# allenai/gpv-1

Measured on AMD Instinct MI355X. Metric: images/sec/node (train step, 480x640, bs32/GPU), higher is better.
Workload: dtype bf16; 1 GPU; GPV-1 (ResNet-50 + 6+6 DETR layers, 100 queries, RoI head, BERT-base, 3 co-attention, 3 text-decoder layers, V=10000) CocoCaptioning-only train step, dropout 0.1, AdamW; global_batch=32, image=480x640, parallelism=dp1

## Files before the change

gpv-1_amd/csrc/gemm_glds_tt.hip:

```cpp
#include "gemm_common.h"

namespace gpvk {
namespace {


typedef __attribute__((address_space(3))) void lds_void_t;
typedef const __attribute__((address_space(1))) void glb_void_t;

__device__ __forceinline__ bf16x8 tr_frag(const unsigned char* p) {
  typedef short __attribute__((ext_vector_type(4))) s16x4;
  typedef __attribute__((address_space(3))) s16x4 lds_s16x4;
  s16x4 a = __builtin_amdgcn_ds_read_tr16_b64_v4i16((lds_s16x4*)(p));
  s16x4 b = __builtin_amdgcn_ds_read_tr16_b64_v4i16((lds_s16x4*)(p + 4 * ROWBYTES));
  typedef short __attribute__((ext_vector_type(8))) s16x8;
  s16x8 r = {a[0], a[1], a[2], a[3], b[0], b[1], b[2], b[3]};
  return __builtin_bit_cast(bf16x8, r);
}

template <bool CONV, int ABL = 0>
__device__ __forceinline__ void glds_tt_core(const GemmK& p, int tile, int ksplit) {
  extern __shared__ __attribute__((aligned(256))) unsigned char smem[];
  const int tid = threadIdx.x, lane = tid & 63, wave = tid >> 6;
  const int wm = wave >> 1, wn = wave & 1;
  const ConvGeom& g = p.cg;
  const int tm = tile / p.tilesN, tn = tile - tm * p.tilesN;
  const int row0 = tm * TBM, col0 = tn * TBN;
  const int kt_total = (p.K + TBK - 1) / TBK;
  const int kt0 = ksplit * p.kt_per_split;
  const int kt1 = min(kt_total, kt0 + p.kt_per_split);
  if (kt0 >= kt1) return;

  int c0 = 0, dh = 0, dw = 0;
  if constexpr (CONV) {
    const int tap = col0 / g.Cin;
    c0 = col0 - tap * g.Cin;
    const int tap_r = tap / g.KW, tap_s = tap - tap_r * g.KW;
    dh = tap_r - g.PH; dw = tap_s - g.PW;
  }

  int px_b = 0, px_oh = 0, px_ow = 0, adv_q = 0, adv_r = 0;
  if constexpr (CONV) {
    const int k = kt0 * TBK + lane;
    px_b = k / (g.OH * g.OW);
    const int rem = k - px_b * (g.OH * g.OW);
    px_oh = rem / g.OW;
    px_ow = rem - px_oh * g.OW;
    adv_q = TBK / g.OW; adv_r = TBK - adv_q * g.OW;
  }

  constexpr int OOB = 0x7ffffff0;
  const int lrow = lane >> 4;
  const int chunk01 = (lane & 15) ^ (2 * lrow);
  const auto rsA = __builtin_amdgcn_make_buffer_rsrc(const_cast<void*>(p.A), (short)0, OOB, 0x00020000);
  const auto rsB = __builtin_amdgcn_make_buffer_rsrc(const_cast<void*>(p.B), (short)0, OOB, 0x00020000);
  int a_vo[4], b_vo[4];
#pragma unroll
  for (int j = 0; j < 4; ++j) {
    const int r = wave * 16 + j * 4 + lrow;
    const int ch = chunk01 ^ ((j >> 1) * 8);
    a_vo[j] = (r * (int)p.lda + row0 + ch * 8) * 2;
    b_vo[j] = CONV ? (c0 + ch * 8) * 2 : (r * (int)p.ldb + col0 + ch * 8) * 2;
  }
  auto bload = [&](const decltype(rsA)& rs, int voff, int soff, unsigned char* l) {
    __builtin_amdgcn_raw_ptr_buffer_load_lds(rs, (lds_void_t*)l, 16, voff, soff, 0, 0);
  };

  auto issue = [&](int kt, int stage) {
    unsigned char* sa = smem + stage * TSTAGE + wave * (4 * 1024);
    unsigned char* sb = sa + OP_BYTES;
    const bool full = (kt + 1) * TBK <= p.K;
    if constexpr (CONV) {
      int off;
      {
        const int ih = px_oh * g.SH + dh, iw = px_ow * g.SW + dw;
        const bool ok = (unsigned)ih < (unsigned)g.IH && (unsigned)iw < (unsigned)g.IW && kt * TBK + lane < p.K;
        off = ok ? ((px_b * g.IH + ih) * g.IW + iw) * g.Cs * 2 : OOB;
        px_ow += adv_r;
        const int c = px_ow >= g.OW ? 1 : 0;
        px_ow -= c ? g.OW : 0;
        px_oh += adv_q + c;
        const int c2 = px_oh >= g.OH ? 1 : 0;
        px_oh -= c2 ? g.OH : 0;
        px_b += c2;
      }
#pragma unroll
      for (int j = 0; j < 4; ++j)
        bload(rsB, __shfl(off, wave * 16 + j * 4 + lrow) + b_vo[j], 0, sb + j * 1024);
    } else {
#pragma unroll
      for (int j = 0; j < 4; ++j) {
        const bool ok = full || kt * TBK + wave * 16 + j * 4 + lrow < p.K;
        bload(rsB, ok ? b_vo[j] : OOB, kt * TBK * (int)p.ldb * 2, sb + j * 1024);
      }
    }
#pragma unroll
    for (int j = 0; j < 4; ++j) {
      const bool ok = full || kt * TBK + wave * 16 + j * 4 + lrow < p.K;
      bload(rsA, ok ? a_vo[j] : OOB, kt * TBK * (int)p.lda * 2, sa + j * 1024);
    }
  };

  f32x4 acc[4][4];
#pragma unroll
  for (int i = 0; i < 4; ++i)
#pragma unroll
    for (int j = 0; j < 4; ++j) acc[i][j] = f32x4{0.f, 0.f, 0.f, 0.f};

  const int li = lane & 15, fg = lane >> 4;
  const int fq = (li >> 2) | ((fg & 1) << 2);
  const int f_row = (8 * fg + (li >> 2)) * ROWBYTES + ((li & 3) >> 1) * 16 + (li & 1) * 8;
  int a_sl[4], b_sl[4];
#pragma unroll
  for (int i = 0; i < 4; ++i) {
    a_sl[i] = f_row + (((wm * 4 + i) ^ fq) << 5);
// ... 4 lines not shown
  f32x4 sacc[4];
#pragma unroll
  for (int i = 0; i < 4; ++i) sacc[i] = f32x4{0.f, 0.f, 0.f, 0.f};
  bf16x8 ones;
#pragma unroll
  for (int e = 0; e < 8; ++e) ones[e] = (bf16)1.0f;

  if (ABL == 5 || ABL == 6) {
    constexpr int AHEAD = ABL == 5 ? 2 : 3;
    for (int a = 0; a < AHEAD && kt0 + a < kt1; ++a) issue(kt0 + a, a & 1);
    for (int kt = kt0; kt < kt1; ++kt) {
      if (ABL == 5) asm volatile("s_waitcnt vmcnt(8)" ::: "memory"); else asm volatile("s_waitcnt vmcnt(16)" ::: "memory");
      __syncthreads();
      if (kt + AHEAD < kt1) issue(kt + AHEAD, kt & 1);
    }
    asm volatile("s_waitcnt vmcnt(0)" ::: "memory");
    return;
  }
  if (ABL != 3) issue(kt0, 0);
  for (int kt = kt0; kt < kt1; ++kt) {
    const int t = kt - kt0;
    asm volatile("s_waitcnt vmcnt(0)" ::: "memory");
    __syncthreads();
    if (ABL != 3 && kt + 1 < kt1) issue(ABL == 4 ? kt0 : kt + 1, (t + 1) & 1);
    const unsigned char* st = smem + (t & 1) * TSTAGE;
    if (ABL == 2 || ABL == 4) continue;
#pragma unroll
    for (int kk = 0; kk < 2; ++kk) {
      bf16x8 af[4], bfr[4];
#pragma unroll
      for (int j = 0; j < 4; ++j) bfr[j] = tr_frag(st + b_sl[j] + kk * 32 * ROWBYTES);
#pragma unroll
      for (int i = 0; i < 4; ++i) af[i] = tr_frag(st + a_sl[i] + kk * 32 * ROWBYTES);
      if (ABL == 1) {
#pragma unroll
        for (int i = 0; i < 4; ++i) asm volatile("" ::"v"(af[i]), "v"(bfr[i]));
        continue;
      }
#pragma unroll
      for (int i = 0; i < 4; ++i)
#pragma unroll
        for (int j = 0; j < 4; ++j) acc[i][j] = mfma16(bfr[j], af[i], acc[i][j]);
      if constexpr (!CONV) {
        if (do_sum) {
#pragma unroll
          for (int i = 0; i < 4; ++i) sacc[i] = mfma16(ones, af[i], sacc[i]);
        }
      }
    }
  }
  if constexpr (!CONV) {
    if (do_sum && fg == 0) {
#pragma unroll
      for (int i = 0; i < 4; ++i) atomicAdd(p.a_rowsum + row0 + wm * 64 + i * 16 + li, sacc[i][0]);
    }
  }

  const bool direct = p.ws == nullptr;
  float* Cp = direct ? reinterpret_cast<float*>(p.C) : p.ws + (int64_t)ksplit * p.M * p.N;
  const int64_t cpitch = direct ? p.ldc : p.N;
  float* ep = reinterpret_cast<float*>(smem);
  constexpr int EPITCH = TBN + 4;
#pragma unroll
  for (int half = 0; half < 2; ++half) {
    __syncthreads();
    if (wm == half) {
#pragma unroll
      for (int i = 0; i < 4; ++i)
#pragma unroll
        for (int j = 0; j < 4; ++j)
          *reinterpret_cast<f32x4*>(ep + (i * 16 + li) * EPITCH + wn * 64 + j * 16 + fg * 4) = acc[i][j];
    }
    __syncthreads();
#pragma unroll
    for (int q = 0; q < 8; ++q) {
      const int idx = tid + q * 256;
      const int r = idx >> 5, c4 = idx & 31;
      const int m = row0 + half * 64 + r;
      if (m >= p.M) continue;
      const float rs = p.rowscale ? p.rowscale[m] * p.alpha : p.alpha;
      float4 v = *reinterpret_cast<const float4*>(ep + r * EPITCH + c4 * 4);
      v.x *= rs; v.y *= rs; v.z *= rs; v.w *= rs;
      float4* dst = reinterpret_cast<float4*>(Cp + (int64_t)m * cpitch + col0 + c4 * 4);
      if (direct) { const float4 c = *dst; v.x += c.x; v.y += c.y; v.z += c.z; v.w += c.w; }
      *dst = v;
    }
  }
}

constexpr int W8_HALF = TBK * ROWBYTES;
constexpr int W8_BUF = 4 * W8_HALF;
constexpr int W8_LDS = 2 * W8_BUF;

typedef short __attribute__((ext_vector_type(4))) w8_s16x4;
typedef short __attribute__((ext_vector_type(8))) w8_s16x8;
template <int OFF>
__device__ __forceinline__ bf16x8 tr_frag_asm(uint32_t addr) {
  w8_s16x4 a, b;
  asm volatile("ds_read_b64_tr_b16 %0, %1 offset:%2" : "=v"(a) : "v"(addr), "n"(OFF) : "memory");
  asm volatile("ds_read_b64_tr_b16 %0, %1 offset:%2" : "=v"(b) : "v"(addr), "n"(OFF + 4 * ROWBYTES) : "memory");
  w8_s16x8 r = {a[0], a[1], a[2], a[3], b[0], b[1], b[2], b[3]};
  return __builtin_bit_cast(bf16x8, r);
}

template <bool CONV>
__device__ __forceinline__ void wg8_core(const GemmK& p, int tile, int ksplit) {
  extern __shared__ __attribute__((aligned(256))) unsigned char smem[];
  const int tid = threadIdx.x, lane = tid & 63;
  const int wave = __builtin_amdgcn_readfirstlane(tid >> 6);
  const int wm = wave >> 2, wn = wave & 3;
  const ConvGeom& g = p.cg;
  const int tm = tile / p.tilesN, tn = tile - tm * p.tilesN;
  const int row0 = tm * 256, col0 = tn * 256;
  const int kt_total = (p.K + TBK - 1) / TBK;
  const int kt0 = ksplit * p.kt_per_split;
  const int kt1 = min(kt_total, kt0 + p.kt_per_split);
  if (kt0 >= kt1) return;
  const int nkt = kt1 - kt0;

  constexpr int OOB = 0x7ffffff0;
  const int lrow = lane >> 4;
  const int myrow = wave * 8 + lrow;
  const int chunk = (lane & 15) ^ (2 * lrow) ^ (8 * (wave & 1));

  int c0 = 0, dh = 0, dw = 0, adv_q = 0, adv_r = 0;
  int px_b[2] = {0, 0}, px_oh[2] = {0, 0}, px_ow[2] = {0, 0}, px_k[2] = {0, 0};
  if constexpr (CONV) {
    const int tap = col0 / g.Cin;
    c0 = col0 - tap * g.Cin;
    const int tap_r = tap / g.KW, tap_s = tap - tap_r * g.KW;
    dh = tap_r - g.PH; dw = tap_s - g.PW;
    adv_q = TBK / g.OW; adv_r = TBK - adv_q * g.OW;
// ... 344 lines not shown
    __builtin_amdgcn_sched_barrier(0);
    issue01(t + 2, buf2);
    asm volatile("s_waitcnt vmcnt(10)" ::: "memory");
    mma(0, 0);
    if constexpr (BH == 2) { W8H_READ_B(2) } else { W8H_READ_A(2) }
    __builtin_amdgcn_sched_barrier(0);
    issue2(t + 2, buf2);
    asm volatile("s_waitcnt vmcnt(8)" ::: "memory");
    if constexpr (BH == 2) mma(0, 2); else mma(4, 0);
    buf = buf == 2 ? 0 : buf + 1;
    buf2 = buf2 == 2 ? 0 : buf2 + 1;
  }
#undef W8H_READ_A
#undef W8H_READ_B
  if (wm == 0) __builtin_amdgcn_s_barrier();
  asm volatile("s_waitcnt vmcnt(0)" ::: "memory");

  const bool direct = p.ws == nullptr;
  float* Cp = direct ? reinterpret_cast<float*>(p.C) : p.ws + (int64_t)ksplit * p.M * p.N;
  const int64_t cpitch = direct ? p.ldc : p.N;
#pragma unroll
  for (int i = 0; i < NI; ++i) {
    const int m = row0 + (i >> 2) * 128 + wm * 64 + (i & 3) * 16 + li;
    const float rs = p.rowscale ? p.rowscale[m] * p.alpha : p.alpha;
#pragma unroll
    for (int j = 0; j < NJ; ++j) {
      if (!hval[j >> 1]) continue;
      const int n = col0 + (j >> 1) * 128 + wn * 32 + (j & 1) * 16 + fg * 4;
      float4* dst = reinterpret_cast<float4*>(Cp + (int64_t)m * cpitch + n);
      float4 v = make_float4(acc[i][j][0] * rs, acc[i][j][1] * rs, acc[i][j][2] * rs, acc[i][j][3] * rs);
      if (direct) { const float4 c = *dst; v.x += c.x; v.y += c.y; v.z += c.z; v.w += c.w; }
      *dst = v;
    }
  }
}

template <bool CONV>
__device__ __forceinline__ void glds_tt_body(const GemmK& p) {
  const int gx = gridDim.x, nwg = gx * (int)gridDim.y, bid = (int)blockIdx.x + gx * (int)blockIdx.y;
  const int v = xcd_contiguous(bid, nwg);
  const int ksplit = v / gx;
  glds_tt_core<CONV>(p, v - ksplit * gx, ksplit);
}
__global__ __launch_bounds__(256) void glds_wgrad_kernel(GemmK p) { glds_tt_body<true>(p); }
__global__ __launch_bounds__(256) void glds_tt_kernel(GemmK p) { glds_tt_body<false>(p); }

struct GroupK {
  int n;
  int tile_start[GPV_TT_GROUP_MAX + 1];
  gpv_tt_problem prob[GPV_TT_GROUP_MAX];
};
static_assert(sizeof(GroupK) <= 4096, "kernel argument segment");

__global__ __launch_bounds__(256) void glds_tt_group_kernel(GroupK g) {
  const int bid = blockIdx.x;
  int pi = 0;
  while (pi + 1 < g.n && bid >= g.tile_start[pi + 1]) ++pi;
  const gpv_tt_problem& q = g.prob[pi];
  GemmK p{};
  p.A = q.A; p.B = q.B; p.C = q.C; p.a_rowsum = q.a_rowsum;
  p.M = q.M; p.N = q.N; p.K = q.K; p.lda = q.lda; p.ldb = q.ldb; p.ldc = q.ldc;
  p.alpha = 1.0f; p.ws = nullptr;
  p.tilesN = q.N / TBN;
  p.kt_per_split = (q.K + TBK - 1) / TBK;
  glds_tt_core<false>(p, bid - g.tile_start[pi], 0);
}

struct WgProb {
  const void* A; const void* B; float* C; const float* rowscale;
  int M, N, K, lda, ldc;
  int kt_per_split, tilesN, tiles;
  int unit_start;
  int direct;
  int64_t ws_off;
  int IH, IW, Cs, Cin, OH, OW, KH, KW, SH, SW, PH, PW;
};
static_assert(sizeof(WgProb) == 128, "descriptor size");
constexpr int WG_MAX = 28;
struct WgGroupK { int n; int pad; float* ws; WgProb prob[WG_MAX]; };
static_assert(sizeof(WgGroupK) <= 4096, "kernel argument segment");

template <int ABL>
__device__ __forceinline__ void wgrad_group_body(const WgGroupK& g) {
  const int nwg = gridDim.x, bid = blockIdx.x;
  const int v = xcd_contiguous(bid, nwg);
  int pi = 0;
  while (pi + 1 < g.n && v >= g.prob[pi + 1].unit_start) ++pi;
  const WgProb& q = g.prob[pi];
  GemmK p{};
  p.A = q.A; p.B = q.B; p.C = q.C; p.rowscale = q.rowscale;
  p.M = q.M; p.N = q.N; p.K = q.K; p.lda = q.lda; p.ldb = 0; p.ldc = q.ldc;
  p.alpha = 1.0f;
  p.ws = q.direct ? nullptr : g.ws + q.ws_off;
  p.tilesN = q.tilesN; p.kt_per_split = q.kt_per_split;
  p.cg.IH = q.IH; p.cg.IW = q.IW; p.cg.Cs = q.Cs; p.cg.Cin = q.Cin; p.cg.OH = q.OH; p.cg.OW = q.OW;
  p.cg.KH = q.KH; p.cg.KW = q.KW; p.cg.SH = q.SH; p.cg.SW = q.SW; p.cg.PH = q.PH; p.cg.PW = q.PW;
  const int u = v - q.unit_start;
  const int ksplit = u / q.tiles;
  glds_tt_core<true, ABL>(p, u - ksplit * q.tiles, ksplit);
}
__global__ __launch_bounds__(256) void glds_wgrad_group_kernel(WgGroupK g) { wgrad_group_body<0>(g); }
__global__ __launch_bounds__(512) void wg8_group_kernel(WgGroupK g) {
  const int nwg = gridDim.x, bid = blockIdx.x;
  const int v = xcd_contiguous(bid, nwg);
  int pi = 0;
  while (pi + 1 < g.n && v >= g.prob[pi + 1].unit_start) ++pi;
  const WgProb& q = g.prob[pi];
  GemmK p{};
  p.A = q.A; p.B = q.B; p.C = q.C; p.rowscale = q.rowscale;
  p.M = q.M; p.N = q.N; p.K = q.K; p.lda = q.lda; p.ldb = 0; p.ldc = q.ldc;
  p.alpha = 1.0f;
  p.ws = q.direct ? nullptr : g.ws + q.ws_off;
  p.tilesN = q.tilesN; p.kt_per_split = q.kt_per_split;
  p.cg.IH = q.IH; p.cg.IW = q.IW; p.cg.Cs = q.Cs; p.cg.Cin = q.Cin; p.cg.OH = q.OH; p.cg.OW = q.OW;
  p.cg.KH = q.KH; p.cg.KW = q.KW; p.cg.SH = q.SH; p.cg.SW = q.SW; p.cg.PH = q.PH; p.cg.PW = q.PW;
  const int u = v - q.unit_start;
  const int ksplit = u / q.tiles;
  wg8_core<true>(p, u - ksplit * q.tiles, ksplit);
}
__global__ __launch_bounds__(512) void wg8h_group_kernel(WgGroupK g) {
  const int nwg = gridDim.x, bid = blockIdx.x;
  const int v = xcd_contiguous(bid, nwg);
  int pi = 0;
  while (pi + 1 < g.n && v >= g.prob[pi + 1].unit_start) ++pi;
  const WgProb& q = g.prob[pi];
  GemmK p{};
  p.A = q.A; p.B = q.B; p.C = q.C; p.rowscale = q.rowscale;
  p.M = q.M; p.N = q.N; p.K = q.K; p.lda = q.lda; p.ldb = 0; p.ldc = q.ldc;
  p.alpha = 1.0f;
  p.ws = (q.direct & 1) ? nullptr : g.ws + q.ws_off;
  p.tilesN = q.tilesN; p.kt_per_split = q.kt_per_split;
  p.cg.IH = q.IH; p.cg.IW = q.IW; p.cg.Cs = q.Cs; p.cg.Cin = q.Cin; p.cg.OH = q.OH; p.cg.OW = q.OW;
  p.cg.KH = q.KH; p.cg.KW = q.KW; p.cg.SH = q.SH; p.cg.SW = q.SW; p.cg.PH = q.PH; p.cg.PW = q.PW;
  const int u = v - q.unit_start;
  const int ksplit = u / q.tiles;
  if (q.direct & 2) wg8h_core<2, 1>(p, u - ksplit * q.tiles, ksplit);
  else wg8h_core<1, 2>(p, u - ksplit * q.tiles, ksplit);
}
#ifdef GPV_TUNING
__global__ __launch_bounds__(256) void glds_wgrad_group_abl1_kernel(WgGroupK g) { wgrad_group_body<1>(g); }
__global__ __launch_bounds__(256) void glds_wgrad_group_abl2_kernel(WgGroupK g) { wgrad_group_body<2>(g); }
__global__ __launch_bounds__(256) void glds_wgrad_group_abl3_kernel(WgGroupK g) { wgrad_group_body<3>(g); }
__global__ __launch_bounds__(256) void glds_wgrad_group_abl4_kernel(WgGroupK g) { wgrad_group_body<4>(g); }
__global__ __launch_bounds__(256) void glds_wgrad_group_abl5_kernel(WgGroupK g) { wgrad_group_body<5>(g); }
__global__ __launch_bounds__(256) void glds_wgrad_group_abl6_kernel(WgGroupK g) { wgrad_group_body<6>(g); }
#endif

constexpr int W8L_PMAX = GPV_TT_GROUP_MAX, W8L_GMAX = 200;
struct W8LProb {
  const void* A; const void* B; float* C; float* a_rowsum;
  int MN, N, K, lda, ldb, ldc;
  int kt_per_split;
  int ws_off;
};
struct W8LGrp { unsigned short v_start; unsigned char prob, slice; };
struct W8LGroupK { int n_prob, n_grp, Q, pad; int cnt[8]; float* ws; W8LProb prob[W8L_PMAX]; W8LGrp grp[W8L_GMAX]; };
static_assert(sizeof(W8LProb) == 64 && sizeof(W8LGrp) == 4 && sizeof(W8LGroupK) <= 4096, "kernel argument segment");

__global__ __launch_bounds__(512) void wg8_tt_group_kernel(W8LGroupK g) {
  const int bid = blockIdx.x, xcd = bid & 7, loc = bid >> 3;
  if (loc >= g.cnt[xcd]) return;
  const int v = xcd * g.Q + loc;
  int lo = 0, hi = g.n_grp - 1;
  while (lo < hi) {
    const int mid = (lo + hi + 1) >> 1;
    if ((int)g.grp[mid].v_start <= v) lo = mid; else hi = mid - 1;
  }
  const W8LGrp gr = g.grp[lo];
  const W8LProb& q = g.prob[gr.prob];
  GemmK p{};
  p.A = q.A; p.B = q.B; p.C = q.C; p.a_rowsum = q.a_rowsum;
  p.M = q.MN / q.N; p.N = q.N; p.K = q.K; p.lda = q.lda; p.ldb = q.ldb; p.ldc = q.ldc;
  p.alpha = 1.0f;
  p.ws = q.ws_off < 0 ? nullptr : g.ws + q.ws_off;
  p.tilesN = q.N / 256; p.kt_per_split = q.kt_per_split;
  wg8_core<false>(p, v - gr.v_start, gr.slice);
}

struct WgRed { const float* ws; float* C; int64_t MN; int split, N, ldc, blk_start; };
struct WgRedK { int n; int pad; WgRed r[WG_MAX]; };

__global__ __launch_bounds__(256) void wgrad_group_reduce_kernel(WgRedK g) {
  const int bid = blockIdx.x;
  int pi = 0;
  while (pi + 1 < g.n && bid >= g.r[pi + 1].blk_start) ++pi;
  const WgRed& q = g.r[pi];
  const int64_t idx = (int64_t)(bid - q.blk_start) * 256 + threadIdx.x;
  if (idx * 4 >= q.MN) return;
  const int nq = q.N >> 2;
  const int m = (int)(idx / nq), c4 = (int)(idx - (int64_t)m * nq);
  const float* src = q.ws + (int64_t)m * q.N + c4 * 4;
  float4 a = {0.f, 0.f, 0.f, 0.f};
#pragma unroll 4
  for (int sidx = 0; sidx < q.split; ++sidx) {
    const float4 v = *reinterpret_cast<const float4*>(src + (int64_t)sidx * q.MN);
    a.x += v.x; a.y += v.y; a.z += v.z; a.w += v.w;
  }
  float4* dst = reinterpret_cast<float4*>(q.C + (int64_t)m * q.ldc + c4 * 4);
  float4 c = *dst;
  c.x += a.x; c.y += a.y; c.z += a.z; c.w += a.w;
  *dst = c;
}

template <typename F>
int launch_tt(F fn, const GemmK& k, const Route& r, bool& attr_done, hipStream_t st) {
  GemmK p = k;
  p.kt_per_split = r.kt_per_split;
  p.ws = reinterpret_cast<float*>(k.ws_base);
  p.tilesN = r.tilesN;
  if (!attr_done) {
    hipError_t e = hipFuncSetAttribute(reinterpret_cast<const void*>(fn), hipFuncAttributeMaxDynamicSharedMemorySize, (int)r.lds);
    if (e != hipSuccess) { (void)hipGetLastError(); return (int)e; }
    attr_done = true;
  }
  hipLaunchKernelGGL(fn, dim3(r.gx, r.gy, r.gz), dim3(r.block), (size_t)r.lds, st, p);
  GPV_CHECK_LAUNCH();
  return launch_splitk_reduce(p.ws, r.split, p.M, p.N, reinterpret_cast<float*>(p.C), p.ldc, st);
}

}

int glds_tt_launch(const GemmK& k, const Route& r, hipStream_t st) {
  static bool attr_done[2] = {false, false};
  if (r.family == FAM_GLDS_WGRAD) return launch_tt(glds_wgrad_kernel, k, r, attr_done[0], st);
  return launch_tt(glds_tt_kernel, k, r, attr_done[1], st);
}

}

extern "C" int gpv_gemm_tt_group(const gpv_tt_problem* problems, int n, void* stream) {
  using namespace gpvk;
  if (!problems || n <= 0) return (int)hipErrorInvalidValue;
  static bool attr_done = false;
  constexpr int lds = 2 * TSTAGE;
  if (!attr_done) {
    hipError_t e = hipFuncSetAttribute(reinterpret_cast<const void*>(glds_tt_group_kernel), hipFuncAttributeMaxDynamicSharedMemorySize, lds);
    if (e != hipSuccess) { (void)hipGetLastError(); return (int)e; }
    attr_done = true;
  }
  for (int i0 = 0; i0 < n; i0 += GPV_TT_GROUP_MAX) {
    GroupK g{};
    g.n = n - i0 < GPV_TT_GROUP_MAX ? n - i0 : GPV_TT_GROUP_MAX;
    int tiles = 0;
    for (int i = 0; i < g.n; ++i) {
      const gpv_tt_problem& q = problems[i0 + i];
      if (!q.A || !q.B || !q.C || q.M <= 0 || q.N <= 0 || q.K <= 0 || q.M % TBM != 0 || q.N % TBN != 0 || q.lda % 8 != 0 ||
          q.ldb % 8 != 0 || q.ldc % 4 != 0 || !al16(q.A) || !al16(q.B) || !al16(q.C) ||
          (int64_t)q.K * q.lda >= (1ll << 30) || (int64_t)q.K * q.ldb >= (1ll << 30))
        return (int)hipErrorInvalidValue;
      g.prob[i] = q;
      g.tile_start[i] = tiles;
      tiles += (q.M / TBM) * (q.N / TBN);
    }
    g.tile_start[g.n] = tiles;
    hipLaunchKernelGGL(glds_tt_group_kernel, dim3(tiles), dim3(256), lds, reinterpret_cast<hipStream_t>(stream), g);
    GPV_CHECK_LAUNCH();
  }
  return 0;
}

extern "C" int gpv_conv_wgrad_group(const gpv_conv_wgrad_problem* probs, int n, void* workspace, int64_t workspace_bytes, void* stream) {
  using namespace gpvk;
  if (!probs || n <= 0) return (int)hipErrorInvalidValue;
  hipStream_t st = reinterpret_cast<hipStream_t>(stream);
  static const int target_kt = [] { const int v = tune_env("GPV_WGRAD_GROUP_KT", 150); return v < 8 ? 8 : v; }();
  static bool attr_done = false;
  constexpr int lds = 2 * TSTAGE;
  typedef void (*wg_fn)(WgGroupK);
#ifdef GPV_TUNING
  static const int abl = tune_env("GPV_WG_ABL", 0);
  const wg_fn fn = abl == 1 ? glds_wgrad_group_abl1_kernel : abl == 2 ? glds_wgrad_group_abl2_kernel : abl == 3 ? glds_wgrad_group_abl3_kernel : abl == 4 ? glds_wgrad_group_abl4_kernel : abl == 5 ? glds_wgrad_group_abl5_kernel : abl == 6 ? glds_wgrad_group_abl6_kernel
                                                                                                        : glds_wgrad_group_kernel;
#else
  const wg_fn fn = glds_wgrad_group_kernel;
#endif
  if (!attr_done) {
    hipError_t e = hipFuncSetAttribute(reinterpret_cast<const void*>(fn), hipFuncAttributeMaxDynamicSharedMemorySize, lds);
    if (e != hipSuccess) { (void)hipGetLastError(); return (int)e; }
    attr_done = true;
  }
  static bool attr8_done = false;
  if (!attr8_done) {
    hipError_t e = hipFuncSetAttribute(reinterpret_cast<const void*>(wg8_group_kernel), hipFuncAttributeMaxDynamicSharedMemorySize, W8_LDS);
    if (e != hipSuccess) { (void)hipGetLastError(); return (int)e; }
    attr8_done = true;
  }
  static const int target_kt8 = [] { const int v = tune_env("GPV_WG8_KT", 150); return v < 8 ? 8 : v; }();
  auto eligible8 = [&](const gpv_conv_wgrad_problem& q) {
    const int64_t K64 = (int64_t)q.B * q.OH * q.OW;
    return q.Cout % 256 == 0 && q.Cin % 256 == 0 && q.Cs % 8 == 0 && al16(q.dy) && al16(q.x) && al16(q.dw) &&
           TBK / q.OW + 2 <= q.OH && (int64_t)q.IH * q.IW * q.Cs * q.B < (1ll << 30) && K64 * q.Cout < (1ll << 30) && K64 >= 8 * TBK;
  };
  static bool attr8h_done = false;
  if (!attr8h_done) {
    hipError_t e = hipFuncSetAttribute(reinterpret_cast<const void*>(wg8h_group_kernel), hipFuncAttributeMaxDynamicSharedMemorySize, W8H_LDS);
    if (e != hipSuccess) { (void)hipGetLastError(); return (int)e; }
    attr8h_done = true;
  }
  static const int forced_kt8h = tune_env("GPV_WG8H_KT", 0);
  static const int ramp_kt8h = tune_env("GPV_WG8H_C", 15);
  auto eligible8h = [&](const gpv_conv_wgrad_problem& q) {
    const int64_t K64 = (int64_t)q.B * q.OH * q.OW;
    return g_knobs.wg8h != 0 && q.Cout % 128 == 0 && q.Cin % 128 == 0 && q.Cs % 8 == 0 && al16(q.dy) && al16(q.x) && al16(q.dw) &&
           TBK / q.OW + 2 <= q.OH && (int64_t)q.IH * q.IW * q.Cs * q.B < (1ll << 30) && K64 * q.Cout < (1ll << 30) && K64 >= 8 * TBK;
  };
  bool use8 = g_knobs.wg8 != 0;
  if (use8 && g_knobs.wg8 == 1) {
    int64_t u8 = 0;
    for (int i = 0; i < n; ++i) {
// ... 77 lines not shown
      e = gpv_conv2d(&a, stream);
      if (e) return e;
      continue;
    }
    const bool big = use8 && eligible8(q);
    const bool half = !big && eligible8h(q);
    const bool tall = half && M % 256 == 0;
    const int tbm = big ? 256 : half ? (tall ? 256 : 128) : TBM, tbn = big ? 256 : half ? (tall ? 128 : 256) : TBN;
    const int K = (int)K64;
    const int kt_total = (K + TBK - 1) / TBK;
    const int tkt = big ? target_kt8 : half ? target_kt8h : target_kt;
    int split = (kt_total + tkt / 2) / tkt;
    if (split < 1) split = 1;
    const int64_t MN = (int64_t)M * N;
    while (split > 1 && (int64_t)split * MN > ws_floats) --split;
    const int kps = (kt_total + split - 1) / split;
    split = (kt_total + kps - 1) / kps;
    WgGroupK& gg = big ? g8 : half ? gh : g;
    if (gg.n == WG_MAX || (split > 1 && (rk.n == WG_MAX || ws_used + (int64_t)split * MN > ws_floats))) {
      const int e = flush();
      if (e) return e;
    }
    int& uu = big ? units8 : half ? unitsh : units;
    WgProb& d = gg.prob[gg.n];
    d.A = q.dy; d.B = q.x; d.C = q.dw; d.rowscale = q.rowscale;
    d.M = M; d.N = N; d.K = K; d.lda = M; d.ldc = N;
    d.kt_per_split = kps; d.tilesN = (N + tbn - 1) / tbn; d.tiles = (M / tbm) * d.tilesN;
    d.unit_start = uu; d.direct = (split == 1 ? 1 : 0) | (tall ? 2 : 0); d.ws_off = ws_used;
    d.IH = q.IH; d.IW = q.IW; d.Cs = q.Cs; d.Cin = q.Cin; d.OH = q.OH; d.OW = q.OW;
    d.KH = q.KH; d.KW = q.KW; d.SH = q.SH; d.SW = q.SW; d.PH = q.PH; d.PW = q.PW;
    uu += d.tiles * split;
    if (split > 1) {
      WgRed& r = rk.r[rk.n];
      r.ws = reinterpret_cast<const float*>(workspace) + ws_used; r.C = q.dw; r.MN = MN; r.split = split; r.N = N; r.ldc = N;
      r.blk_start = rblocks;
      rblocks += (int)((MN / 4 + 255) / 256);
      ++rk.n;
      ws_used += (int64_t)split * MN;
    }
    ++gg.n;
  }
  return flush();
}

extern "C" int gpv_gemm_tt_group_ws(const gpv_tt_problem* problems, int n, void* workspace, int64_t workspace_bytes, void* stream) {
  using namespace gpvk;
  if (!problems || n <= 0) return (int)hipErrorInvalidValue;
  hipStream_t st = reinterpret_cast<hipStream_t>(stream);
  static const int target_kt = [] { const int v = tune_env("GPV_W8L_KT", 48); return v < 8 ? 8 : v; }();
  static bool attr_done = false;
  if (!attr_done) {
    hipError_t e = hipFuncSetAttribute(reinterpret_cast<const void*>(wg8_tt_group_kernel), hipFuncAttributeMaxDynamicSharedMemorySize, W8_LDS);
    if (e != hipSuccess) { (void)hipGetLastError(); return (int)e; }
    attr_done = true;
  }
  const int64_t ws_floats = workspace ? workspace_bytes / 4 : 0;
  gpv_tt_problem rest[GPV_TT_GROUP_MAX];
  int n_rest = 0;
  auto flush_rest = [&]() -> int {
    if (n_rest == 0) return 0;
    const int e = gpv_gemm_tt_group(rest, n_rest, stream);
    n_rest = 0;
    return e;
  };
  struct Grp { int prob, slice, tiles, kps; };
  W8LGroupK g{};
  WgRedK rk{};
  Grp grp[W8L_GMAX];
  int n_grp = 0, rblocks = 0;
  int64_t ws_used = 0;
  auto flush = [&]() -> int {
    if (g.n_prob == 0) return 0;
    for (int i = 1; i < n_grp; ++i) {
      const Grp x = grp[i];
      int j = i - 1;
      while (j >= 0 && grp[j].kps < x.kps) { grp[j + 1] = grp[j]; --j; }
      grp[j + 1] = x;
    }
    int64_t load[8] = {0, 0, 0, 0, 0, 0, 0, 0};
    int bin_of[W8L_GMAX], cnt[8] = {0, 0, 0, 0, 0, 0, 0, 0};
    for (int i = 0; i < n_grp; ++i) {
      int b = 0;
      for (int x = 1; x < 8; ++x) if (load[x] < load[b]) b = x;
      bin_of[i] = b;
      load[b] += (int64_t)grp[i].tiles * grp[i].kps;
      cnt[b] += grp[i].tiles;
    }
    int Q = 0;
    for (int x = 0; x < 8; ++x) { g.cnt[x] = cnt[x]; if (cnt[x] > Q) Q = cnt[x]; }
    if (8 * Q >= 65536) return (int)hipErrorInvalidValue;
    g.Q = Q; g.n_grp = n_grp;
    int k = 0;
    for (int x = 0; x < 8; ++x) {
      int off = 0;
      for (int i = 0; i < n_grp; ++i) {
        if (bin_of[i] != x) continue;
        g.grp[k].v_start = (unsigned short)(x * Q + off); g.grp[k].prob = (unsigned char)grp[i].prob; g.grp[k].slice = (unsigned char)grp[i].slice;
        off += grp[i].tiles;
        ++k;
      }
    }
    g.ws = reinterpret_cast<float*>(workspace);
    hipLaunchKernelGGL(wg8_tt_group_kernel, dim3(8 * Q), dim3(512), W8_LDS, st, g);
    GPV_CHECK_LAUNCH();
    ++g_knobs.n_wg8;
    if (rk.n > 0) {
      hipLaunchKernelGGL(wgrad_group_reduce_kernel, dim3(rblocks), dim3(256), 0, st, rk);
      GPV_CHECK_LAUNCH();
    }
    g.n_prob = 0; n_grp = 0; rk.n = 0; rblocks = 0; ws_used = 0;
    return 0;
  };
  for (int i = 0; i < n; ++i) {
    const gpv_tt_problem& q = problems[i];
    const bool big = g_knobs.w8l != 0 && q.A && q.B && q.C && q.M > 0 && q.N > 0 && q.M % 256 == 0 && q.N % 256 == 0 && q.K >= 2 * TBK && (int64_t)q.M * q.N < (1ll << 30) &&
                     q.lda % 8 == 0 && q.ldb % 8 == 0 && q.ldc % 4 == 0 && al16(q.A) && al16(q.B) && al16(q.C) &&
                     (int64_t)q.K * q.lda < (1ll << 30) && (int64_t)q.K * q.ldb < (1ll << 30);
    if (!big) {
      if (n_rest == GPV_TT_GROUP_MAX) { const int e = flush_rest(); if (e) return e; }
      rest[n_rest++] = q;
      continue;
    }
    const int kt_total = (q.K + TBK - 1) / TBK;
    int split = (kt_total + target_kt / 2) / target_kt;
    if (split < 1) split = 1;
    const int64_t MN = (int64_t)q.M * q.N;
    while (split > 1 && (int64_t)split * MN > ws_floats) --split;
    const int kps = (kt_total + split - 1) / split;
    split = (kt_total + kps - 1) / kps;
    if (split > 255) return (int)hipErrorInvalidValue;
    if (g.n_prob == W8L_PMAX || n_grp + split > W8L_GMAX || ws_used + (int64_t)split * MN >= (1ll << 31) || (split > 1 && (rk.n == WG_MAX || ws_used + (int64_t)split * MN > ws_floats))) {
      const int e = flush();
      if (e) return e;
    }
    W8LProb& d = g.prob[g.n_prob];
    d.A = q.A; d.B = q.B; d.C = q.C; d.a_rowsum = q.a_rowsum;
    d.MN = (int)MN; d.N = q.N; d.K = q.K; d.lda = q.lda; d.ldb = q.ldb; d.ldc = q.ldc;
    d.kt_per_split = kps; d.ws_off = split == 1 ? -1 : (int)ws_used;
    const int tiles = (q.M / 256) * (q.N / 256);
    for (int sidx = 0; sidx < split; ++sidx) {
      const int len = (sidx + 1) * kps <= kt_total ? kps : kt_total - sidx * kps;
      grp[n_grp++] = Grp{g.n_prob, sidx, tiles, len};
    }
    if (split > 1) {
      WgRed& r = rk.r[rk.n];
      r.ws = reinterpret_cast<const float*>(workspace) + ws_used; r.C = q.C; r.MN = MN; r.split = split; r.N = q.N; r.ldc = q.ldc;
      r.blk_start = rblocks;
      rblocks += (int)((MN / 4 + 255) / 256);
      ++rk.n;
      ws_used += (int64_t)split * MN;
    }
    ++g.n_prob;
  }
  int e = flush();
  if (e) return e;
  return flush_rest();
}
```

gpv-1_amd/hip.py:

```python
import ctypes as C
import os
import threading

import torch

from . import _native

ABI_VERSION = 2
BF16, F32 = 0, 1
ACT_NONE, ACT_RELU, ACT_GELU = 0, 1, 2
KMAJOR, TRANS = 0, 1

_LIB = None
TUNING = os.environ.get('GPV_TUNING_LIB', '0') == '1'
_LIB_PATH = os.environ.get('GPV_HIP_LIB') or (os.path.join(os.path.dirname(_native.lib_path('hip')), 'libgpv_hip_tuning.so') if TUNING
                                               else _native.lib_path('hip'))


class GemmArgs(C.Structure):
    _fields_ = [('A', C.c_void_p), ('B', C.c_void_p), ('C', C.c_void_p),
                ('M', C.c_int), ('N', C.c_int), ('K', C.c_int), ('batch', C.c_int),
                ('lda', C.c_int64), ('ldb', C.c_int64), ('ldc', C.c_int64),
                ('sA', C.c_int64), ('sB', C.c_int64), ('sC', C.c_int64),
                ('layoutA', C.c_int), ('layoutB', C.c_int), ('dtype_in', C.c_int), ('dtype_out', C.c_int),
# ... 183 lines not shown
        raise TypeError('expected fp32 tensor')
    return t


_WS = {}
WS_MAX = 256 << 20
_WS_RETIRED = []


def _workspace(device, nbytes):
    need = min(nbytes, WS_MAX)
    key = (device, _raw_stream(torch.cuda.current_device()) if _raw_stream is not None else 0)
    ws = _WS.get(key)
    if ws is None or ws.numel() < need:
        if ws is not None:
            _WS_RETIRED.append(ws)
            need = max(need, min(2 * ws.numel(), WS_MAX))
        ws = _WS[key] = torch.empty(max(need, 64 << 20), device=device, dtype=torch.uint8)
    return ws


def gemm(A, B, Cm, M, N, K, lda, ldb, ldc, layoutA=KMAJOR, layoutB=KMAJOR, batch=1, sA=0, sB=0, sC=0,
         alpha=1.0, rowscale=None, bias=None, res=None, ldr=0, sR=0, relu_mask=None, ldm=0, act=ACT_NONE,
         drop_p=0.0, seed=0, accumulate=False, split_k=1, a_rowsum=None, kpad_finite=False):
    a = GemmArgs()
    a.A, a.B, a.C = _p(A), _p(B), _p(Cm)
    a.M, a.N, a.K, a.batch = M, N, K, batch
    a.lda, a.ldb, a.ldc, a.sA, a.sB, a.sC = lda, ldb, ldc, sA, sB, sC
    a.layoutA, a.layoutB = layoutA, layoutB
    if A.dtype != B.dtype:
        raise TypeError('gemm: A and B dtypes differ')
    a.dtype_in, a.dtype_out = dcode(A), dcode(Cm)
    a.alpha = alpha
    if rowscale is not None or bias is not None:
        check_epilogue_extents('gemm', M, N, rowscale, bias)
    a.rowscale, a.bias = _p(_f32(rowscale)), _p(_f32(bias))
    if res is not None and res.dtype != Cm.dtype:
        raise TypeError('gemm: residual dtype must equal output dtype')
    if relu_mask is not None and relu_mask.dtype != Cm.dtype:
        raise TypeError('gemm: mask dtype must equal output dtype')
    a.res, a.ldr, a.sR = _p(res), ldr, sR
    a.relu_mask, a.ldm = _p(relu_mask), ldm
    a.act, a.drop_p, a.seed = act, drop_p, seed
    a.accumulate, a.split_k = int(accumulate), split_k
    a.a_rowsum = _p(_f32(a_rowsum))
    a.flags = (1 if kpad_finite else 0) | getattr(_TL, 'gemm_flags', 0)
    if accumulate and batch == 1:
        ws = _workspace(A.device, max(max(split_k, 8) * M * N * 4, 512 * 128 * 128 * 4))
        a.workspace, a.workspace_bytes = _p(ws), ws.numel()
    _chk(lib().gpv_gemm(C.byref(a), _stream()), 'gpv_gemm')


def tt_group_ok(dy, x, dw, M, N, K, lda, ldb, ldc):
    return (dy.dtype == torch.bfloat16 and x.dtype == torch.bfloat16 and dw.dtype == torch.float32 and M % 128 == 0 and N % 128 == 0
            and lda % 8 == 0 and ldb % 8 == 0 and ldc % 4 == 0 and dy.data_ptr() % 16 == 0 and x.data_ptr() % 16 == 0
            and dw.data_ptr() % 16 == 0 and K * max(lda, ldb) < (1 << 30))


def gemm_tt_group(problems):
    if not problems:
        return
    problems = sorted(problems, key=lambda q: -q[6])
    arr = (TTProblem * len(problems))()
    for i, (dy, x, dw, bg, M, N, K, lda, ldb, ldc) in enumerate(problems):
        a = arr[i]
        a.A, a.B, a.C, a.a_rowsum = dy.data_ptr(), x.data_ptr(), dw.data_ptr(), (bg.data_ptr() if bg is not None else None)
        a.M, a.N, a.K, a.lda, a.ldb, a.ldc = M, N, K, lda, ldb, ldc
    if _OPT_SET.get(OPT_W8L, 0) or os.environ.get('GPV_W8L', '0') not in ('', '0'):
        ws = _workspace(problems[0][0].device, WS_MAX)
        _chk(lib().gpv_gemm_tt_group_ws(arr, C.c_int(len(problems)), _p(ws), C.c_int64(ws.numel()), _stream()), 'gpv_gemm_tt_group_ws')
    else:
        _chk(lib().gpv_gemm_tt_group_ws(arr, C.c_int(len(problems)), None, C.c_int64(0), _stream()), 'gpv_gemm_tt_group_ws')


def check_epilogue_extents(what, rows, cols, rowscale, bias):
    if rowscale is not None and rowscale.numel() < rows:
        raise ValueError('%s: rowscale has %d elements, the epilogue indexes it by output row: %d needed' % (what, rowscale.numel(), rows))
    if bias is not None and bias.numel() < cols:
        raise ValueError('%s: bias has %d elements, the epilogue indexes it by output column: %d needed' % (what, bias.numel(), cols))


def _conv_args(mode, x, w, y, B, IH, IW, Cs, Cin, OH, OW, Cout, KH, KW, SH, SW, PH, PW, rowscale=None, bias=None,
               res=None, relu_mask=None, act=ACT_NONE, split_k=0, y_mask_bits=None, relu_mask_bits=None):
    a = ConvArgs()
    a.mode = mode
    a.x, a.w, a.y = _p(x), _p(w), _p(y)
    a.B, a.IH, a.IW, a.Cs, a.Cin, a.OH, a.OW, a.Cout = B, IH, IW, Cs, Cin, OH, OW, Cout
    a.KH, a.KW, a.SH, a.SW, a.PH, a.PW = KH, KW, SH, SW, PH, PW
    a.dtype_in, a.dtype_out = dcode(x), dcode(y)
    if x.dtype != w.dtype:
        raise TypeError('conv2d: operand dtypes differ')
    if rowscale is not None or bias is not None:
        check_epilogue_extents('conv2d mode %d' % mode, Cout if mode == 2 else B * OH * OW, KH * KW * Cin if mode == 2 else Cout, rowscale, bias)
    a.rowscale, a.bias = _p(_f32(rowscale)), _p(_f32(bias))
    for t in (res, relu_mask):
        if t is not None and t.dtype != y.dtype:
            raise TypeError('conv2d: res/mask dtype must equal output dtype')
    a.res, a.relu_mask = _p(res), _p(relu_mask)
    a.act, a.split_k = act, split_k
    for t in (y_mask_bits, relu_mask_bits):
        if t is not None and (t.dtype != torch.int32 or not t.is_contiguous() or t.numel() * 32 != B * OH * OW * Cout):
            raise TypeError('conv2d: mask bits are a contiguous int32 [pixels, Cout / 32] tensor')
    a.y_mask_bits, a.relu_mask_bits = _p(y_mask_bits), _p(relu_mask_bits)
    return a


def conv2d_mask_bits_ok(*args, **kw):
    return bool(lib().gpv_conv2d_mask_bits_ok(C.byref(_conv_args(*args, **kw))))


def conv2d(mode, x, w, y, B, IH, IW, Cs, Cin, OH, OW, Cout, KH, KW, SH, SW, PH, PW, rowscale=None, bias=None,
           res=None, relu_mask=None, act=ACT_NONE, split_k=0, y_mask_bits=None, relu_mask_bits=None):
    a = _conv_args(mode, x, w, y, B, IH, IW, Cs, Cin, OH, OW, Cout, KH, KW, SH, SW, PH, PW, rowscale, bias, res, relu_mask, act, split_k,
                   y_mask_bits, relu_mask_bits)
    if mode == 2:
        ws = _workspace(x.device, WS_MAX)
        a.workspace, a.workspace_bytes = _p(ws), ws.numel()
    elif mode == 0 and B * OH * OW <= 8192 and KH * KW * Cin >= 1024:
        ws = _workspace(x.device, 16 * B * OH * OW * Cout * 4)
        a.workspace, a.workspace_bytes = _p(ws), ws.numel()
    _chk(lib().gpv_conv2d(C.byref(a), _stream()), 'gpv_conv2d')


def conv_wgrad_group(problems):
    if not problems:
# ... 380 lines not shown
```

Before: 2121 images/sec.

## Support ragged M/N in grouped TT weight-grad GEMM and add split-K sliced path

Extends the grouped transposed-transposed (weight-gradient) GEMM kernel so it handles M/N that are multiples of 8 rather than 128, by clamping load offsets and masking stores and rowsum atomics. Problems with ragged shapes that previously fell back to another path can now use the grouped kernels. A new sliced-group kernel also applies split-K to these ragged problems using the existing workspace and reduce machinery, and the Python side now always allocates a workspace. This adds extra launches and a reduce pass, and some clamped loads re-read the same data.

Measured after the change: 2116 images/sec. About the same (-0.3%).

```diff
diff --git a/gpv-1_amd/csrc/gemm_glds_tt.hip b/gpv-1_amd/csrc/gemm_glds_tt.hip
--- a/gpv-1_amd/csrc/gemm_glds_tt.hip
+++ b/gpv-1_amd/csrc/gemm_glds_tt.hip
@@ -17,7 +17,7 @@
   return __builtin_bit_cast(bf16x8, r);
 }
 
-template <bool CONV, int ABL = 0>
+template <bool CONV, int ABL = 0, bool RAG = false>
 __device__ __forceinline__ void glds_tt_core(const GemmK& p, int tile, int ksplit) {
   extern __shared__ __attribute__((aligned(256))) unsigned char smem[];
   const int tid = threadIdx.x, lane = tid & 63, wave = tid >> 6;
@@ -58,8 +58,10 @@
   for (int j = 0; j < 4; ++j) {
     const int r = wave * 16 + j * 4 + lrow;
     const int ch = chunk01 ^ ((j >> 1) * 8);
-    a_vo[j] = (r * (int)p.lda + row0 + ch * 8) * 2;
-    b_vo[j] = CONV ? (c0 + ch * 8) * 2 : (r * (int)p.ldb + col0 + ch * 8) * 2;
+    const int ca = RAG ? min(row0 + ch * 8, p.M - 8) : row0 + ch * 8;
+    const int cb = RAG ? min(col0 + ch * 8, p.N - 8) : col0 + ch * 8;
+    a_vo[j] = (r * (int)p.lda + ca) * 2;
+    b_vo[j] = CONV ? (c0 + ch * 8) * 2 : (r * (int)p.ldb + cb) * 2;
   }
   auto bload = [&](const decltype(rsA)& rs, int voff, int soff, unsigned char* l) {
     __builtin_amdgcn_raw_ptr_buffer_load_lds(rs, (lds_void_t*)l, 16, voff, soff, 0, 0);
@@ -170,7 +172,10 @@
   if constexpr (!CONV) {
     if (do_sum && fg == 0) {
 #pragma unroll
-      for (int i = 0; i < 4; ++i) atomicAdd(p.a_rowsum + row0 + wm * 64 + i * 16 + li, sacc[i][0]);
+      for (int i = 0; i < 4; ++i) {
+        const int m = row0 + wm * 64 + i * 16 + li;
+        if (!RAG || m < p.M) atomicAdd(p.a_rowsum + m, sacc[i][0]);
+      }
     }
   }
 
@@ -196,6 +201,7 @@
       const int r = idx >> 5, c4 = idx & 31;
       const int m = row0 + half * 64 + r;
       if (m >= p.M) continue;
+      if (RAG && col0 + c4 * 4 >= p.N) continue;
       const float rs = p.rowscale ? p.rowscale[m] * p.alpha : p.alpha;
       float4 v = *reinterpret_cast<const float4*>(ep + r * EPITCH + c4 * 4);
       v.x *= rs; v.y *= rs; v.z *= rs; v.w *= rs;
@@ -646,6 +652,7 @@
 };
 static_assert(sizeof(GroupK) <= 4096, "kernel argument segment");
 
+template <bool RAG>
 __global__ __launch_bounds__(256) void glds_tt_group_kernel(GroupK g) {
   const int bid = blockIdx.x;
   int pi = 0;
@@ -655,9 +662,9 @@
   p.A = q.A; p.B = q.B; p.C = q.C; p.a_rowsum = q.a_rowsum;
   p.M = q.M; p.N = q.N; p.K = q.K; p.lda = q.lda; p.ldb = q.ldb; p.ldc = q.ldc;
   p.alpha = 1.0f; p.ws = nullptr;
-  p.tilesN = q.N / TBN;
+  p.tilesN = (q.N + TBN - 1) / TBN;
   p.kt_per_split = (q.K + TBK - 1) / TBK;
-  glds_tt_core<false>(p, bid - g.tile_start[pi], 0);
+  glds_tt_core<false, 0, RAG>(p, bid - g.tile_start[pi], 0);
 }
 
 struct WgProb {
@@ -751,9 +758,10 @@
 struct W8LGroupK { int n_prob, n_grp, Q, pad; int cnt[8]; float* ws; W8LProb prob[W8L_PMAX]; W8LGrp grp[W8L_GMAX]; };
 static_assert(sizeof(W8LProb) == 64 && sizeof(W8LGrp) == 4 && sizeof(W8LGroupK) <= 4096, "kernel argument segment");
 
-__global__ __launch_bounds__(512) void wg8_tt_group_kernel(W8LGroupK g) {
+template <int TILE>
+__device__ __forceinline__ bool w8l_unit(const W8LGroupK& g, GemmK& p, int& tile, int& slice) {
   const int bid = blockIdx.x, xcd = bid & 7, loc = bid >> 3;
-  if (loc >= g.cnt[xcd]) return;
+  if (loc >= g.cnt[xcd]) return false;
   const int v = xcd * g.Q + loc;
   int lo = 0, hi = g.n_grp - 1;
   while (lo < hi) {
@@ -762,13 +770,24 @@
   }
   const W8LGrp gr = g.grp[lo];
   const W8LProb& q = g.prob[gr.prob];
-  GemmK p{};
   p.A = q.A; p.B = q.B; p.C = q.C; p.a_rowsum = q.a_rowsum;
   p.M = q.MN / q.N; p.N = q.N; p.K = q.K; p.lda = q.lda; p.ldb = q.ldb; p.ldc = q.ldc;
   p.alpha = 1.0f;
   p.ws = q.ws_off < 0 ? nullptr : g.ws + q.ws_off;
-  p.tilesN = q.N / 256; p.kt_per_split = q.kt_per_split;
-  wg8_core<false>(p, v - gr.v_start, gr.slice);
+  p.tilesN = (q.N + TILE - 1) / TILE; p.kt_per_split = q.kt_per_split;
+  tile = v - gr.v_start; slice = gr.slice;
+  return true;
+}
+
+__global__ __launch_bounds__(512) void wg8_tt_group_kernel(W8LGroupK g) {
+  GemmK p{};
+  int tile, slice;
+  if (w8l_unit<256>(g, p, tile, slice)) wg8_core<false>(p, tile, slice);
+}
+__global__ __launch_bounds__(256) void glds_tt_sliced_group_kernel(W8LGroupK g) {
+  GemmK p{};
+  int tile, slice;
+  if (w8l_unit<TBM>(g, p, tile, slice)) glds_tt_core<false, 0, true>(p, tile, slice);
 }
 
 struct WgRed { const float* ws; float* C; int64_t MN; int split, N, ldc, blk_start; };
@@ -812,6 +831,13 @@
   return launch_splitk_reduce(p.ws, r.split, p.M, p.N, reinterpret_cast<float*>(p.C), p.ldc, st);
 }
 
+inline bool tt_problem_ok(const gpv_tt_problem& q) {
+  return q.A && q.B && q.C && q.M > 0 && q.N > 0 && q.K > 0 && q.M % 8 == 0 && q.N % 8 == 0 && q.lda % 8 == 0 && q.ldb % 8 == 0 &&
+         q.ldc % 4 == 0 && al16(q.A) && al16(q.B) && al16(q.C) &&
+         (int64_t)q.K * q.lda < (1ll << 30) && (int64_t)q.K * q.ldb < (1ll << 30);
+}
+inline int tt_tiles(const gpv_tt_problem& q) { return ((q.M + TBM - 1) / TBM) * ((q.N + TBN - 1) / TBN); }
+
 }
 
 int glds_tt_launch(const GemmK& k, const Route& r, hipStream_t st) {
@@ -828,27 +854,30 @@
   static bool attr_done = false;
   constexpr int lds = 2 * TSTAGE;
   if (!attr_done) {
-    hipError_t e = hipFuncSetAttribute(reinterpret_cast<const void*>(glds_tt_group_kernel), hipFuncAttributeMaxDynamicSharedMemorySize, lds);
+    hipError_t e = hipFuncSetAttribute(reinterpret_cast<const void*>(glds_tt_group_kernel<false>), hipFuncAttributeMaxDynamicSharedMemorySize, lds);
+    if (e != hipSuccess) { (void)hipGetLastError(); return (int)e; }
+    e = hipFuncSetAttribute(reinterpret_cast<const void*>(glds_tt_group_kernel<true>), hipFuncAttributeMaxDynamicSharedMemorySize, lds);
     if (e != hipSuccess) { (void)hipGetLastError(); return (int)e; }
     attr_done = true;
   }
-  for (int i0 = 0; i0 < n; i0 += GPV_TT_GROUP_MAX) {
+  for (int i = 0; i < n; ++i)
+    if (!tt_problem_ok(problems[i])) return (int)hipErrorInvalidValue;
+  for (int rag = 0; rag < 2; ++rag) {
     GroupK g{};
-    g.n = n - i0 < GPV_TT_GROUP_MAX ? n - i0 : GPV_TT_GROUP_MAX;
     int tiles = 0;
-    for (int i = 0; i < g.n; ++i) {
-      const gpv_tt_problem& q = problems[i0 + i];
-      if (!q.A || !q.B || !q.C || q.M <= 0 || q.N <= 0 || q.K <= 0 || q.M % TBM != 0 || q.N % TBN != 0 || q.lda % 8 != 0 ||
-          q.ldb % 8 != 0 || q.ldc % 4 != 0 || !al16(q.A) || !al16(q.B) || !al16(q.C) ||
-          (int64_t)q.K * q.lda >= (1ll << 30) || (int64_t)q.K * q.ldb >= (1ll << 30))
-        return (int)hipErrorInvalidValue;
-      g.prob[i] = q;
-      g.tile_start[i] = tiles;
-      tiles += (q.M / TBM) * (q.N / TBN);
-    }
-    g.tile_start[g.n] = tiles;
-    hipLaunchKernelGGL(glds_tt_group_kernel, dim3(tiles), dim3(256), lds, reinterpret_cast<hipStream_t>(stream), g);
-    GPV_CHECK_LAUNCH();
+    for (int i = 0; i <= n; ++i) {
+      if (i < n && (((problems[i].M | problems[i].N) & (TBM - 1)) != 0) != (rag != 0)) continue;
+      if (g.n == GPV_TT_GROUP_MAX || (i == n && g.n > 0)) {
+        g.tile_start[g.n] = tiles;
+        hipLaunchKernelGGL(rag ? glds_tt_group_kernel<true> : glds_tt_group_kernel<false>, dim3(tiles), dim3(256), lds, reinterpret_cast<hipStream_t>(stream), g);
+        GPV_CHECK_LAUNCH();
+        g.n = 0; tiles = 0;
+      }
+      if (i == n) break;
+      g.prob[g.n] = problems[i];
+      g.tile_start[g.n++] = tiles;
+      tiles += tt_tiles(problems[i]);
+    }
   }
   return 0;
 }
@@ -1032,9 +1061,22 @@
   if (!attr_done) {
     hipError_t e = hipFuncSetAttribute(reinterpret_cast<const void*>(wg8_tt_group_kernel), hipFuncAttributeMaxDynamicSharedMemorySize, W8_LDS);
     if (e != hipSuccess) { (void)hipGetLastError(); return (int)e; }
+    e = hipFuncSetAttribute(reinterpret_cast<const void*>(glds_tt_sliced_group_kernel), hipFuncAttributeMaxDynamicSharedMemorySize, 2 * TSTAGE);
+    if (e != hipSuccess) { (void)hipGetLastError(); return (int)e; }
     attr_done = true;
   }
   const int64_t ws_floats = workspace ? workspace_bytes / 4 : 0;
+  constexpr int SL_KT = 8, SL_UNITS = 256;
+  auto slices128 = [&](const gpv_tt_problem& q) {
+    const int kt_total = (q.K + TBK - 1) / TBK, tiles = tt_tiles(q);
+    int split = (kt_total + SL_KT / 2) / SL_KT;
+    if (split > SL_UNITS / tiles) split = SL_UNITS / tiles;
+    if (split > 255) split = 255;
+    return split < 1 ? 1 : split;
+  };
+  int kind = 0;
+  for (int i = 0; i < n; ++i)
+    if (!tt_problem_ok(problems[i])) return (int)hipErrorInvalidValue;
   gpv_tt_problem rest[GPV_TT_GROUP_MAX];
   int n_rest = 0;
   auto flush_rest = [&]() -> int {
@@ -1081,9 +1123,14 @@
       }
     }
     g.ws = reinterpret_cast<float*>(workspace);
-    hipLaunchKernelGGL(wg8_tt_group_kernel, dim3(8 * Q), dim3(512), W8_LDS, st, g);
-    GPV_CHECK_LAUNCH();
-    ++g_knobs.n_wg8;
+    if (kind == 0) {
+      hipLaunchKernelGGL(wg8_tt_group_kernel, dim3(8 * Q), dim3(512), W8_LDS, st, g);
+      GPV_CHECK_LAUNCH();
+      ++g_knobs.n_wg8;
+    } else {
+      hipLaunchKernelGGL(glds_tt_sliced_group_kernel, dim3(8 * Q), dim3(256), 2 * TSTAGE, st, g);
+      GPV_CHECK_LAUNCH();
+    }
     if (rk.n > 0) {
       hipLaunchKernelGGL(wgrad_group_reduce_kernel, dim3(rblocks), dim3(256), 0, st, rk);
       GPV_CHECK_LAUNCH();
@@ -1091,48 +1138,55 @@
     g.n_prob = 0; n_grp = 0; rk.n = 0; rblocks = 0; ws_used = 0;
     return 0;
   };
-  for (int i = 0; i < n; ++i) {
-    const gpv_tt_problem& q = problems[i];
-    const bool big = g_knobs.w8l != 0 && q.A && q.B && q.C && q.M > 0 && q.N > 0 && q.M % 256 == 0 && q.N % 256 == 0 && q.K >= 2 * TBK && (int64_t)q.M * q.N < (1ll << 30) &&
-                     q.lda % 8 == 0 && q.ldb % 8 == 0 && q.ldc % 4 == 0 && al16(q.A) && al16(q.B) && al16(q.C) &&
-                     (int64_t)q.K * q.lda < (1ll << 30) && (int64_t)q.K * q.ldb < (1ll << 30);
-    if (!big) {
-      if (n_rest == GPV_TT_GROUP_MAX) { const int e = flush_rest(); if (e) return e; }
-      rest[n_rest++] = q;
-      continue;
-    }
+  auto plan = [&](const gpv_tt_problem& q, int& split) {
+    const int64_t MN = (int64_t)q.M * q.N;
     const int kt_total = (q.K + TBK - 1) / TBK;
-    int split = (kt_total + target_kt / 2) / target_kt;
+    const bool big = g_knobs.w8l != 0 && q.M % 256 == 0 && q.N % 256 == 0 && q.K >= 2 * TBK && MN < (1ll << 30);
+    split = big ? (kt_total + target_kt / 2) / target_kt : ((q.M | q.N) & (TBM - 1)) != 0 ? slices128(q) : 1;
     if (split < 1) split = 1;
-    const int64_t MN = (int64_t)q.M * q.N;
     while (split > 1 && (int64_t)split * MN > ws_floats) --split;
-    const int kps = (kt_total + split - 1) / split;
-    split = (kt_total + kps - 1) / kps;
-    if (split > 255) return (int)hipErrorInvalidValue;
-    if (g.n_prob == W8L_PMAX || n_grp + split > W8L_GMAX || ws_used + (int64_t)split * MN >= (1ll << 31) || (split > 1 && (rk.n == WG_MAX || ws_used + (int64_t)split * MN > ws_floats))) {
-      const int e = flush();
-      if (e) return e;
-    }
-    W8LProb& d = g.prob[g.n_prob];
-    d.A = q.A; d.B = q.B; d.C = q.C; d.a_rowsum = q.a_rowsum;
-    d.MN = (int)MN; d.N = q.N; d.K = q.K; d.lda = q.lda; d.ldb = q.ldb; d.ldc = q.ldc;
-    d.kt_per_split = kps; d.ws_off = split == 1 ? -1 : (int)ws_used;
-    const int tiles = (q.M / 256) * (q.N / 256);
-    for (int sidx = 0; sidx < split; ++sidx) {
-      const int len = (sidx + 1) * kps <= kt_total ? kps : kt_total - sidx * kps;
-      grp[n_grp++] = Grp{g.n_prob, sidx, tiles, len};
-    }
-    if (split > 1) {
-      WgRed& r = rk.r[rk.n];
-      r.ws = reinterpret_cast<const float*>(workspace) + ws_used; r.C = q.C; r.MN = MN; r.split = split; r.N = q.N; r.ldc = q.ldc;
-      r.blk_start = rblocks;
-      rblocks += (int)((MN / 4 + 255) / 256);
-      ++rk.n;
-      ws_used += (int64_t)split * MN;
-    }
-    ++g.n_prob;
-  }
-  int e = flush();
-  if (e) return e;
+    return big ? 0 : split > 1 && MN < (1ll << 30) ? 1 : 2;
+  };
+  for (kind = 0; kind < 2; ++kind) {
+    for (int i = 0; i < n; ++i) {
+      const gpv_tt_problem& q = problems[i];
+      int split;
+      const int where = plan(q, split);
+      if (where == 2 && kind == 0) {
+        if (n_rest == GPV_TT_GROUP_MAX) { const int e = flush_rest(); if (e) return e; }
+        rest[n_rest++] = q;
+      }
+      if (where != kind) continue;
+      const int kt_total = (q.K + TBK - 1) / TBK;
+      const int64_t MN = (int64_t)q.M * q.N;
+      const int kps = (kt_total + split - 1) / split;
+      split = (kt_total + kps - 1) / kps;
+      if (split > 255) return (int)hipErrorInvalidValue;
+      if (g.n_prob == W8L_PMAX || n_grp + split > W8L_GMAX || ws_used + (int64_t)split * MN >= (1ll << 31) || (split > 1 && (rk.n == WG_MAX || ws_used + (int64_t)split * MN > ws_floats))) {
+        const int e = flush();
+        if (e) return e;
+      }
+      W8LProb& d = g.prob[g.n_prob];
+      d.A = q.A; d.B = q.B; d.C = q.C; d.a_rowsum = q.a_rowsum;
+      d.MN = (int)MN; d.N = q.N; d.K = q.K; d.lda = q.lda; d.ldb = q.ldb; d.ldc = q.ldc;
+      d.kt_per_split = kps; d.ws_off = split == 1 ? -1 : (int)ws_used;
+      const int tiles = kind == 0 ? (q.M / 256) * (q.N / 256) : tt_tiles(q);
+      for (int sidx = 0; sidx < split; ++sidx) {
+        const int len = (sidx + 1) * kps <= kt_total ? kps : kt_total - sidx * kps;
+        grp[n_grp++] = Grp{g.n_prob, sidx, tiles, len};
+      }
+      if (split > 1) {
+        WgRed& r = rk.r[rk.n];
+        r.ws = reinterpret_cast<const float*>(workspace) + ws_used; r.C = q.C; r.MN = MN; r.split = split; r.N = q.N; r.ldc = q.ldc;
+        r.blk_start = rblocks;
+        rblocks += (int)((MN / 4 + 255) / 256);
+        ++rk.n;
+        ws_used += (int64_t)split * MN;
+      }
+      ++g.n_prob;
+    }
+    const int e = flush();
+    if (e) return e;
+  }
   return flush_rest();
 }
diff --git a/gpv-1_amd/hip.py b/gpv-1_amd/hip.py
--- a/gpv-1_amd/hip.py
+++ b/gpv-1_amd/hip.py
@@ -259,7 +259,7 @@
 
 
 def tt_group_ok(dy, x, dw, M, N, K, lda, ldb, ldc):
-    return (dy.dtype == torch.bfloat16 and x.dtype == torch.bfloat16 and dw.dtype == torch.float32 and M % 128 == 0 and N % 128 == 0
+    return (dy.dtype == torch.bfloat16 and x.dtype == torch.bfloat16 and dw.dtype == torch.float32 and M % 8 == 0 and N % 8 == 0
             and lda % 8 == 0 and ldb % 8 == 0 and ldc % 4 == 0 and dy.data_ptr() % 16 == 0 and x.data_ptr() % 16 == 0
             and dw.data_ptr() % 16 == 0 and K * max(lda, ldb) < (1 << 30))
 
@@ -277,7 +277,8 @@
         ws = _workspace(problems[0][0].device, WS_MAX)
         _chk(lib().gpv_gemm_tt_group_ws(arr, C.c_int(len(problems)), _p(ws), C.c_int64(ws.numel()), _stream()), 'gpv_gemm_tt_group_ws')
     else:
-        _chk(lib().gpv_gemm_tt_group_ws(arr, C.c_int(len(problems)), None, C.c_int64(0), _stream()), 'gpv_gemm_tt_group_ws')
+        ws = _workspace(problems[0][0].device, 64 << 20)
+        _chk(lib().gpv_gemm_tt_group_ws(arr, C.c_int(len(problems)), _p(ws), C.c_int64(ws.numel()), _stream()), 'gpv_gemm_tt_group_ws')
 
 
 def check_epilogue_extents(what, rows, cols, rowscale, bias):
```
